# google-research/nerf-from-image

Measured on AMD Instinct MI355X. Metric: rendered rays/sec (128x128, 64+64 samples), higher is better.
Workload: dtype f32 (decoder MLP operands split-fp16 hi+lo, 22 bits; strict fp32: config.value_mlp_exact_fp32)

## Files before the change

nerf_from_image_amd/csrc/nfi_device.hpp:

```cpp
#pragma once
#include <hip/hip_runtime.h>
#include <stdint.h>

#ifndef NFI_RENDER_OCC
#define NFI_RENDER_OCC 2
#endif

namespace nfi {

typedef float f32x4 __attribute__((ext_vector_type(4)));
typedef unsigned int u32x4 __attribute__((ext_vector_type(4)));
typedef _Float16 f16x8 __attribute__((ext_vector_type(8)));

constexpr int kWave = 64;
constexpr int kC = 32;
constexpr int kHidden = 64;
constexpr float kLog2e = 1.4426950408889634f;
constexpr float kLn2 = 0.6931471805599453f;
constexpr float kSoftplusThr2 = 28.853900817779268f;

constexpr int kW1F = 0;
constexpr int kW2F = kW1F + 8 * 64 * 4;
constexpr int kB1F = kW2F + 4 * 64 * 4;
constexpr int kB2F = kB1F + 64;
// ... 659 lines not shown
            if (row >= 1 && row <= A) q[(row - 1) * (-SEMP)] = (unsigned short)(int)pq;
          } else {
            if (row >= 1 && row <= A) sem[n][row - 1] = e4[r] * inv;
          }
        }
      }
    } else {
      float r1 = bcast_row0(o[n].y), r2 = bcast_row0(o[n].z), r3 = bcast_row0(o[n].w);
      res[n].r = (1.0f / (1.0f + __builtin_amdgcn_exp2f(-r1))) * 2.004f - 1.002f;
      res[n].g = (1.0f / (1.0f + __builtin_amdgcn_exp2f(-r2))) * 2.004f - 1.002f;
      res[n].b = (1.0f / (1.0f + __builtin_amdgcn_exp2f(-r3))) * 2.004f - 1.002f;
    }
  }
}

__device__ __forceinline__ void split_f16x8(const float (&x)[8], f16x8& hi, f16x8& lo) {
  typedef float f32x2 __attribute__((ext_vector_type(2)));
#pragma unroll
  for (int i = 0; i < 4; ++i) {
    auto h = __builtin_amdgcn_cvt_pkrtz(x[2 * i], x[2 * i + 1]);
    float r0, r1;
    const uint32_t hb = __builtin_bit_cast(uint32_t, h);
    asm("v_fma_mix_f32 %0, -%1, 1.0, %2 op_sel:[0,0,0] op_sel_hi:[1,0,0]" : "=v"(r0) : "v"(hb), "v"(x[2 * i]));
    asm("v_fma_mix_f32 %0, -%1, 1.0, %2 op_sel:[1,0,0] op_sel_hi:[1,0,0]" : "=v"(r1) : "v"(hb), "v"(x[2 * i + 1]));
    auto l = __builtin_amdgcn_cvt_pkrtz(r0, r1);
    hi[2 * i] = h[0]; hi[2 * i + 1] = h[1];
    lo[2 * i] = l[0]; lo[2 * i + 1] = l[1];
  }
}

// ... 53 lines not shown
    const f16x8 al = __builtin_bit_cast(f16x8, w1t[((0 * 2 + kk) * 2 + 1) * 64 + lane]);
    const f16x8 bh = __builtin_bit_cast(f16x8, w1t[((1 * 2 + kk) * 2 + 0) * 64 + lane]);
    const f16x8 bl = __builtin_bit_cast(f16x8, w1t[((1 * 2 + kk) * 2 + 1) * 64 + lane]);
    const f32x4 zero = {0.0f, 0.0f, 0.0f, 0.0f};
    G[kk][0] = __builtin_amdgcn_mfma_f32_16x16x32_f16(al, sh, zero, 0, 0, 0);
    G[kk][1] = __builtin_amdgcn_mfma_f32_16x16x32_f16(bl, sh, zero, 0, 0, 0);
    G[kk][0] = __builtin_amdgcn_mfma_f32_16x16x32_f16(ah, sl, G[kk][0], 0, 0, 0);
    G[kk][1] = __builtin_amdgcn_mfma_f32_16x16x32_f16(bh, sl, G[kk][1], 0, 0, 0);
    G[kk][0] = __builtin_amdgcn_mfma_f32_16x16x32_f16(ah, sh, G[kk][0], 0, 0, 0);
    G[kk][1] = __builtin_amdgcn_mfma_f32_16x16x32_f16(bh, sh, G[kk][1], 0, 0, 0);
  }
  const f32x4 G0 = G[0][0] + G[1][0], G1 = G[0][1] + G[1][1];
  Gout0 = G0; Gout1 = G1;
}

template <bool ATT, int N, int PREC, int SEMP = 0, bool NRM = false>
__device__ __forceinline__ void tile_mlp(const FieldParams& P, int lane, const float (&feat)[N][8],
                                         const float (&outside)[N], float* const (&sem)[N], TileOut (&res)[N],
                                         f32x4 (&Gout)[N][2]) {
  const int g = lane >> 4;
  const f32x4* ldsv = reinterpret_cast<const f32x4*>(P.lds);
  f32x4 o[N];
  if constexpr (PREC == 1) {
    const u32x4* ldsu = reinterpret_cast<const u32x4*>(P.lds);
    f16x8 fh[N], fl[N];
#pragma unroll
    for (int n = 0; n < N; ++n) split_f16x8(feat[n], fh[n], fl[n]);
    f32x4 acc1[N][4];
#pragma unroll
    for (int nt = 0; nt < 4; ++nt) {
      const f32x4 b = ldsv[(kB1F >> 2) + g * 4 + nt];
      const f16x8 wh = __builtin_bit_cast(f16x8, ldsu[(kW1H_lds >> 2) + (nt * 2 + 0) * 64 + lane]);
      const f16x8 wl = __builtin_bit_cast(f16x8, ldsu[(kW1H_lds >> 2) + (nt * 2 + 1) * 64 + lane]);
#pragma unroll
      for (int n = 0; n < N; ++n) acc1[n][nt] = __builtin_amdgcn_mfma_f32_16x16x32_f16(wh, fh[n], b, 0, 0, 0);
#pragma unroll
      for (int n = 0; n < N; ++n) acc1[n][nt] = __builtin_amdgcn_mfma_f32_16x16x32_f16(wh, fl[n], acc1[n][nt], 0, 0, 0);
// ... 76 lines not shown
    for (int n = 0; n < N; ++n) { o0[n] = b2; o1[n] = f32x4{0.0f, 0.0f, 0.0f, 0.0f}; }
#pragma unroll
    for (int nt = 0; nt < 4; ++nt) {
      const f32x4 w = ldsv[(kW2F >> 2) + nt * 64 + lane];
#pragma unroll
      for (int n = 0; n < N; ++n) {
        o0[n] = __builtin_amdgcn_mfma_f32_16x16x4f32(w.x, acc1[n][nt][0], o0[n], 0, 0, 0);
        o1[n] = __builtin_amdgcn_mfma_f32_16x16x4f32(w.y, acc1[n][nt][1], o1[n], 0, 0, 0);
        o0[n] = __builtin_amdgcn_mfma_f32_16x16x4f32(w.z, acc1[n][nt][2], o0[n], 0, 0, 0);
        o1[n] = __builtin_amdgcn_mfma_f32_16x16x4f32(w.w, acc1[n][nt][3], o1[n], 0, 0, 0);
      }
    }
#pragma unroll
    for (int n = 0; n < N; ++n) o[n] = o0[n] + o1[n];
  }

  tile_epilogue<ATT, N, SEMP>(P, lane, o, outside, sem, res);
}
template <bool ATT, int N, int PREC, int SEMP = 0>
__device__ __forceinline__ void tile_mlp(const FieldParams& P, int lane, const float (&feat)[N][8],
                                         const float (&outside)[N], float* const (&sem)[N], TileOut (&res)[N]) {
  f32x4 unused[N][2];
  tile_mlp<ATT, N, PREC, SEMP, false>(P, lane, feat, outside, sem, res, unused);
}

template <bool ATT, int N, int SEMP = 0, bool NRM = false>
__device__ __forceinline__ void tile_mlp_vd(const FieldParams& P, int lane, const float (&feat)[N][8],
                                            const f32x4 (&xr)[N][3], const float (&outside)[N], float* const (&sem)[N],
                                            TileOut (&res)[N], f32x4 (&Gout)[N][2]) {
  const int g = lane >> 4;
  const f32x4* ldsv = reinterpret_cast<const f32x4*>(P.lds);
  f32x4 acc1[N][4];
#pragma unroll
  for (int nt = 0; nt < 4; ++nt) {
    const f32x4 b = ldsv[(kVdB1F >> 2) + g * 4 + nt];
#pragma unroll
    for (int n = 0; n < N; ++n) acc1[n][nt] = b;
  }
#pragma unroll
  for (int s = 0; s < 8; ++s) {
    const f32x4 w = ldsv[(kVdW1F >> 2) + s * 64 + lane];
#pragma unroll
    for (int n = 0; n < N; ++n) {
      acc1[n][0] = __builtin_amdgcn_mfma_f32_16x16x4f32(w.x, feat[n][s], acc1[n][0], 0, 0, 0);
// ... 28 lines not shown
    for (int n = 0; n < N; ++n) o2[n][t] = b;
  }
#pragma unroll
  for (int nt = 0; nt < 4; ++nt)
#pragma unroll
    for (int t = 0; t < 3; ++t) {
      const f32x4 w = ldsv[(kVdW2 >> 2) + (t * 4 + nt) * 64 + lane];
#pragma unroll
      for (int n = 0; n < N; ++n) {
        o2[n][t] = __builtin_amdgcn_mfma_f32_16x16x4f32(w.x, acc1[n][nt][0], o2[n][t], 0, 0, 0);
        o2[n][t] = __builtin_amdgcn_mfma_f32_16x16x4f32(w.y, acc1[n][nt][1], o2[n][t], 0, 0, 0);
        o2[n][t] = __builtin_amdgcn_mfma_f32_16x16x4f32(w.z, acc1[n][nt][2], o2[n][t], 0, 0, 0);
        o2[n][t] = __builtin_amdgcn_mfma_f32_16x16x4f32(w.w, acc1[n][nt][3], o2[n][t], 0, 0, 0);
      }
    }
  f32x4 o[N], oB[N];
  const f32x4 b3 = ldsv[(kVdB3 >> 2) + g];
#pragma unroll
  for (int n = 0; n < N; ++n) { o[n] = b3; oB[n] = f32x4{0.0f, 0.0f, 0.0f, 0.0f}; }
#pragma unroll
  for (int t = 0; t < 3; ++t) {
    const f32x4 w = ldsv[(kVdW3 >> 2) + t * 64 + lane];
#pragma unroll
    for (int n = 0; n < N; ++n) {
      f32x4 y;
#pragma unroll
      for (int r = 0; r < 4; ++r) {
        const float v = o2[n][t][r] + xr[n][t][r];
        y[r] = (v >= 0.0f) ? v : v * 0.2f;
      }
      if (t == 0 && g == 0) y[0] = o2[n][0][0];
      o[n] = __builtin_amdgcn_mfma_f32_16x16x4f32(w.x, y[0], o[n], 0, 0, 0);
      oB[n] = __builtin_amdgcn_mfma_f32_16x16x4f32(w.y, y[1], oB[n], 0, 0, 0);
      o[n] = __builtin_amdgcn_mfma_f32_16x16x4f32(w.z, y[2], o[n], 0, 0, 0);
      oB[n] = __builtin_amdgcn_mfma_f32_16x16x4f32(w.w, y[3], oB[n], 0, 0, 0);
    }
  }
#pragma unroll
  for (int n = 0; n < N; ++n) o[n] = o[n] + oB[n];
  tile_epilogue<ATT, N, SEMP>(P, lane, o, outside, sem, res);
}

struct SampleOut {
  float sdf, sigma, r, g, b;
  float nx, ny, nz;
};

template <int TEX, bool ATT, bool SKIP, int PREC = 0, bool VD = false, int SEMP = 0, bool NRM = false>
__device__ __forceinline__ SampleOut field_wave(const FieldParams& P, float scene_range, int lane, float px, float py,
                                                float pz, bool valid, float* sem_base, bool* outside_flag,
                                                float* stage, unsigned long long* prof = nullptr,
                                                const float* xray = nullptr, int ray_idx = 0) {
  float qx = px / scene_range, qy = py / scene_range, qz = pz / scene_range;
  bool out = (fabsf(qx) > 1.0f) || (fabsf(qy) > 1.0f) || (fabsf(qz) > 1.0f);
  if (outside_flag) *outside_flag = out;
  int x0, y0, z0;
  float fx, fy, fz;
  plane_coord(qx, P.res_m1, P.res, x0, fx);
  plane_coord(qy, P.res_m1, P.res, y0, fy);
  plane_coord(qz, P.res_m1, P.res, z0, fz);
  if (!valid) { x0 = y0 = z0 = 0; fx = fy = fz = 0.0f; }
  const int xi = (int)((uint32_t)x0 | ((uint32_t)y0 << 10) | ((uint32_t)z0 << 20));
  int flags = (out ? 1 : 0) | (valid ? 2 : 0);
  if constexpr (NRM) {
    auto inside = [&](float q) { float u = ((q + 1.0f) / 2.0f) * P.res_m1; return (u > 0.0f && u < P.res_m1) ? 1 : 0; };
    flags |= (inside(qx) << 2) | (inside(qy) << 3) | (inside(qz) << 4);
  }
  const uint64_t live = SKIP ? __ballot(valid && !out) : __ballot(valid);
  uint32_t tm = 0;
#pragma unroll
  for (int t = 0; t < 4; ++t) tm |= (((live >> (16 * t)) & 0xFFFFull) != 0 ? 1u : 0u) << t;

  SampleOut so;
  so.sdf = 0.0f; so.sigma = 0.0f; so.r = 0.0f; so.g = 0.0f; so.b = 0.0f;
  so.nx = 0.0f; so.ny = 0.0f; so.nz = 0.0f;
  if (tm == 0) return so;
  const int j = lane & 15, g = lane >> 4;

  const int lp = lane >> 2, lq = lane & 3;
  auto gather_tile = [&](int t, float (&feat)[8]) -> int {
    const int srcL = 16 * t + lp, srcM = 16 * t + j;
    const float cfx = __shfl(fx, srcL, 64), cfy = __shfl(fy, srcL, 64), cfz = __shfl(fz, srcL, 64);
    const uint32_t cxi = (uint32_t)__shfl(xi, srcL, 64);
    const int fcur = __shfl(flags, srcM, 64);
    float featL[8];
    TileTex<TEX> T;
    tile_issue<TEX>(P, lq, cxi, T);
    tile_bilinear<TEX>(T, cfx, cfy, cfz, featL);
    __builtin_amdgcn_sched_barrier(0);
    f32x4* wr = reinterpret_cast<f32x4*>(stage + lp * 36 + lq * 4);
    wr[0] = f32x4{featL[0], featL[1], featL[2], featL[3]};
    wr[4] = f32x4{featL[4], featL[5], featL[6], featL[7]};
    wave_lds_fence();
    const f32x4* rd = reinterpret_cast<const f32x4*>(stage + j * 36 + g * 4);
    const f32x4 lo = rd[0], hi = rd[4];
    feat[0] = lo.x; feat[1] = lo.y; feat[2] = lo.z; feat[3] = lo.w;
    feat[4] = hi.x; feat[5] = hi.y; feat[6] = hi.z; feat[7] = hi.w;
    wave_lds_fence();
    __builtin_amdgcn_sched_barrier(0);
// ... 8 lines not shown
#pragma unroll
    for (int a = 0; a < 3; ++a) {
      gcoord[a] += dpp_f32<kDppQuadXor1>(0.0f, gcoord[a]);
      gcoord[a] += dpp_f32<kDppQuadXor2>(0.0f, gcoord[a]);
    }
    const int flL = __shfl(flags, 16 * t + lp, 64);
    float gx = ((flL >> 2) & 1) ? gcoord[0] : 0.0f, gy = ((flL >> 3) & 1) ? gcoord[1] : 0.0f,
          gz = ((flL >> 4) & 1) ? gcoord[2] : 0.0f;
    const float sc = ((P.res_m1 * 0.5f) / scene_range) * P.w2r0[64];
    gx *= sc; gy *= sc; gz *= sc;
    const float rn = __builtin_amdgcn_rsqf(fmaxf(fmaf(gx, gx, fmaf(gy, gy, gz * gz)), 1e-24f));
    gx *= rn; gy *= rn; gz *= rn;
    const float sx = __shfl(gx, 4 * j, 64), sy = __shfl(gy, 4 * j, 64), sz = __shfl(gz, 4 * j, 64);
    if (g == t) { so.nx = sx; so.ny = sy; so.nz = sz; }
  };
#pragma unroll 1
  while (tm != 0) {
    if constexpr (NRM) {
      int tprev = -1;
      float dL[3][8];
      f32x4 Gp1[2];
      auto normals_of_previous = [&]() {
        f32x4* wr = reinterpret_cast<f32x4*>(stage + j * 36 + g * 4);
        wr[0] = Gp1[0]; wr[4] = Gp1[1];
        wave_lds_fence();
        float gfL[8];
        {
          const f32x4* rd = reinterpret_cast<const f32x4*>(stage + lp * 36 + lq * 4);
          const f32x4 lo = rd[0], hi = rd[4];
          gfL[0] = lo.x; gfL[1] = lo.y; gfL[2] = lo.z; gfL[3] = lo.w;
          gfL[4] = hi.x; gfL[5] = hi.y; gfL[6] = hi.z; gfL[7] = hi.w;
        }
        wave_lds_fence();
// ... 37 lines not shown
        {
          f32x4* wr = reinterpret_cast<f32x4*>(stage + lp * 36 + lq * 4);
          wr[0] = f32x4{featL[0], featL[1], featL[2], featL[3]};
          wr[4] = f32x4{featL[4], featL[5], featL[6], featL[7]};
          wave_lds_fence();
          const f32x4* rd = reinterpret_cast<const f32x4*>(stage + j * 36 + g * 4);
          const f32x4 lo = rd[0], hi = rd[4];
          feat1[0][0] = lo.x; feat1[0][1] = lo.y; feat1[0][2] = lo.z; feat1[0][3] = lo.w;
          feat1[0][4] = hi.x; feat1[0][5] = hi.y; feat1[0][6] = hi.z; feat1[0][7] = hi.w;
          wave_lds_fence();
        }
        __builtin_amdgcn_sched_barrier(0);
        __builtin_amdgcn_s_setprio(0);
        const float outs1[1] = {(f1 & 1) ? 1.0f : 0.0f};
        float* const sems1[1] = {(sem_base && (f1 & 2)) ? sem_col(t) : nullptr};
        TileOut to1[1];
        f32x4 G1[1][2];
        if constexpr (VD) {
          static_assert(PREC == 0, "the view-direction decoder exists in exact fp32 only");
          const int r1 = __shfl(ray_idx, 16 * t + j, 64);
          f32x4 xr1[1][3];
#pragma unroll
          for (int c3 = 0; c3 < 3; ++c3) xr1[0][c3] = *reinterpret_cast<const f32x4*>(xray + (size_t)r1 * kRayFeatPad + 16 * c3 + 4 * g);
          tile_mlp_vd<ATT, 1, SEMP, true>(P, lane, feat1, xr1, outs1, sems1, to1, G1);
        } else {
          tile_mlp<ATT, 1, PREC, SEMP, true>(P, lane, feat1, outs1, sems1, to1, G1);
        }
        Gp1[0] = G1[0][0]; Gp1[1] = G1[0][1];
        tprev = t;
        if (g == t) { so.sdf = to1[0].sdf; so.sigma = to1[0].sigma; so.r = to1[0].r; so.g = to1[0].g; so.b = to1[0].b; }
      }
      if (tprev >= 0) normals_of_previous();
      return so;
    }
    unsigned long long c0 = prof ? __builtin_readcyclecounter() : 0;
    const int ta = __builtin_ctz(tm);
    tm &= tm - 1;
    const bool pair = tm != 0;
    const int tb = pair ? __builtin_ctz(tm) : ta;
    tm &= tm - 1;
    float feat[2][8];
    __builtin_amdgcn_s_setprio(3);
    const int fa = gather_tile(ta, feat[0]);
    int fb = fa;
    if (pair) {
      fb = gather_tile(tb, feat[1]);
    } else {
#pragma unroll
      for (int s8 = 0; s8 < 8; ++s8) feat[1][s8] = feat[0][s8];
    }
    unsigned long long c2 = prof ? __builtin_readcyclecounter() : 0;
    __builtin_amdgcn_s_setprio(0);
    const float outs[2] = {(fa & 1) ? 1.0f : 0.0f, (fb & 1) ? 1.0f : 0.0f};
    float* const sems[2] = {(sem_base && (fa & 2)) ? sem_col(ta) : nullptr, (sem_base && pair && (fb & 2)) ? sem_col(tb) : nullptr};
    TileOut to[2];
    f32x4 Gp[2][2];
    if constexpr (VD) {
      static_assert(PREC == 0, "the view-direction decoder exists in exact fp32 only");
      const int ra = __shfl(ray_idx, 16 * ta + j, 64), rb = __shfl(ray_idx, 16 * tb + j, 64);
      f32x4 xr[2][3];
#pragma unroll
      for (int t = 0; t < 3; ++t) {
        xr[0][t] = *reinterpret_cast<const f32x4*>(xray + (size_t)ra * kRayFeatPad + 16 * t + 4 * g);
        xr[1][t] = *reinterpret_cast<const f32x4*>(xray + (size_t)rb * kRayFeatPad + 16 * t + 4 * g);
      }
      tile_mlp_vd<ATT, 2, SEMP, false>(P, lane, feat, xr, outs, sems, to, Gp);
    } else {
      tile_mlp<ATT, 2, PREC, SEMP, false>(P, lane, feat, outs, sems, to, Gp);
    }
    if (g == ta) { so.sdf = to[0].sdf; so.sigma = to[0].sigma; so.r = to[0].r; so.g = to[0].g; so.b = to[0].b; }
    if (pair && g == tb) { so.sdf = to[1].sdf; so.sigma = to[1].sigma; so.r = to[1].r; so.g = to[1].g; so.b = to[1].b; }
    if (prof) {
      asm volatile("" :: "v"(so.sigma), "v"(so.r));
      unsigned long long c3 = __builtin_readcyclecounter();
      prof[1] += c2 - c0; prof[2] += c3 - c2; prof[3] += pair ? 2 : 1;
    }
  }
  return so;
}

template <int SPL>
__device__ __forceinline__ void ray_weights(const float (&sigma)[SPL], const float (&t)[SPL], int n, float dnorm,
                                            int lane, float (&w)[SPL], float (&T)[SPL]) {
  float tn[SPL], om[SPL], alpha[SPL];
  next_elem<SPL>(t, tn, lane);
#pragma unroll
  for (int j = 0; j < SPL; ++j) {
    int e = j * 64 + lane;
    float delta = (e < n - 1) ? (tn[j] - t[j]) : 0.0f;
    delta = delta * dnorm;
// ... 28 lines not shown
```

nerf_from_image_amd/csrc/nfi_kernels.hip:

```cpp
#include "nfi_device.hpp"
#include "../../include/nfi_hip.h"
#include "nfi_host.hpp"

#include <algorithm>
#include <cstddef>
#include <cstdio>
#include <cstring>

using namespace nfi;

thread_local char nfi_err_buf[256] = "";
extern "C" const char* nfi_last_error(void) { return nfi_err_buf; }
extern "C" int nfi_version(void) { return 102; }


constexpr int kP2tPixels = 256, kP2tPitch = 288;
template <int TEX>
__global__ __launch_bounds__(256) void planes_to_texels_kernel(const float* __restrict__ planes, void* __restrict__ texels,
                                                               int hw) {
  __shared__ __attribute__((aligned(16))) float tile[kC][kP2tPitch];
  const int img = blockIdx.y;
  const int px0 = blockIdx.x * kP2tPixels;
  const float* src = planes + (size_t)img * kC * hw;
  {
// ... 430 lines not shown
  int64_t total = a->n_rays * a->n_samples;
  hipLaunchKernelGGL(stratified_kernel, dim3((unsigned)((total + 255) / 256)), dim3(256), 0, (hipStream_t)stream, *a);
  return check_launch("stratified_points");
}

struct FieldKernelParams {
  const float* points; int64_t P;
  const void* texels; int res; int tex;
  const float* image; int A; const float* att;
  int use_sdf; const float* beta; const float* alpha; float scene_range;
  float* sigma; float* rgb; float* sdf; float* sem; uint8_t* outside;
  const float* xray; int spr;
  int layout;
};

template <int TEX, bool ATT, bool VD = false, int PREC = 0>
__global__ __launch_bounds__(256) void field_query_kernel(FieldKernelParams k) {
  constexpr int kImg = VD ? kVdImageFloats : kLdsImageFloats;
  __shared__ __attribute__((aligned(16))) float lds[kImg + 64];
  __shared__ __attribute__((aligned(16))) float stages[4][16 * 36];
  const int scene = blockIdx.y;
  stage_field_lds(lds, k.image, k.att ? k.att + (size_t)scene * k.A * 3 : nullptr, k.A, kImg);
  if (PREC == 1) {
    __syncthreads();
    for (int i = threadIdx.x; i < kB1F; i += blockDim.x) lds[i] = k.image[kW1H + i];
  }
  __syncthreads();
  const size_t tb = TEX == 0 ? 128 : 64;
  const char* tex_scene = reinterpret_cast<const char*>(k.texels) + (size_t)scene * 3 * k.res * k.res * tb;
  FieldParams P = make_field_params(tex_scene, k.res, TEX, k.A, k.use_sdf, k.beta, k.alpha, lds, kImg, k.layout);
  const int lane = lane_id();
  const int wave = threadIdx.x >> 6;
  const int64_t n_chunks = (k.P + 63) / 64;
  const float* xray_scene = VD ? k.xray + (size_t)scene * (size_t)(k.P / k.spr) * kRayFeatPad : nullptr;
  for (int64_t chunk = (int64_t)blockIdx.x * 4 + wave; chunk < n_chunks; chunk += (int64_t)gridDim.x * 4) {
    int64_t p = chunk * 64 + lane;
    bool valid = p < k.P;
    size_t gi = (size_t)scene * k.P + (valid ? p : 0);
    float px = 0.0f, py = 0.0f, pz = 0.0f;
    if (valid) { px = k.points[gi * 3]; py = k.points[gi * 3 + 1]; pz = k.points[gi * 3 + 2]; }
    bool out;
    float* sem = k.sem ? k.sem + ((size_t)scene * k.P + chunk * 64) * k.A : nullptr;
    SampleOut so = field_wave<TEX, ATT, false, PREC, VD>(P, k.scene_range, lane, px, py, pz, valid, sem, &out, stages[wave],
                                                      nullptr, xray_scene, VD && valid ? (int)(p / k.spr) : 0);
    if (valid) {
      k.sigma[gi] = so.sigma;
      k.rgb[gi * 3] = so.r; k.rgb[gi * 3 + 1] = so.g; k.rgb[gi * 3 + 2] = so.b;
      if (k.sdf) k.sdf[gi] = so.sdf;
      if (k.outside) k.outside[gi] = out ? 1 : 0;
    }
  }
}

static int field_check_call(const nfi_field_args* a) {
  REQUIRE(a && a->points && a->sigma && a->rgb, "field_query: null pointer");
  REQUIRE(a->n_scenes > 0 && a->points_per_scene > 0, "field_query: bad shape");
  int rc = check_field_common(a->texels, a->plane_res, a->texel_dtype, a->decoder_image, a->n_attention,
                              a->attention_values, a->use_sdf, a->beta, a->alpha, a->texel_layout);
  if (rc) return rc;
// ... 986 lines not shown
    if (ends) { nxt = got; return; }
    a = got;
  }
  cur = nxt = a;
}

template <int TEX, bool ATT, int OCC, int MODE, int PREC, bool VD = false>
__global__ __launch_bounds__(256, OCC) void render_fwd_kernel(RenderKernelParams k) {
  constexpr bool TAPS = MODE == kRenderTaps, PROF = MODE == kRenderProf, TERM = MODE == kRenderTerm;
  constexpr bool EXTRA = MODE == kRenderExtra || MODE == kRenderNormals, NRM = MODE == kRenderNormals;
  constexpr int SEMP = (EXTRA && ATT) ? kSemPitch : 0;
  constexpr int kImg = VD ? kVdImageFloats : kLdsImageFloats;
  __shared__ __attribute__((aligned(16))) float lds[kImg];
  __shared__ __attribute__((aligned(16))) float vfs[4][64];
  __shared__ WaveSlab slabs[4];
  if constexpr (NRM) stage_normal_operands(nfi_dyn_lds, k.image, VD ? kVdW1F : kW1F, VD ? kVdW2 : kW2F);
  ClockProbe clock;
  clock.start(k);
  stage_decoder_image<PREC, kImg>(lds, k.image);
  const int lane = lane_id();
  const int wave = threadIdx.x >> 6;
  WaveSlab& slab = slabs[wave];
  float* vf = vfs[wave];
  const int S = k.S;
  const bool valid = lane < S;
  const float fill_near = ordered_key_inv(~k.reduce[0]), fill_far = ordered_key_inv(k.reduce[1]);
  const float bg = k.white ? 1.0f : 0.0f;
  const uint32_t n_rays = (uint32_t)k.n_scenes * (uint32_t)k.hw;

  FieldParams P = make_field_params(k.texels, k.res, TEX, k.A, k.use_sdf, k.beta, k.alpha, lds, kImg, k.layout);
  P.vf = vf;
  P.w1t = nfi_dyn_lds; P.w2r0 = nfi_dyn_lds + kW1TFloats;
  int cur_scene = -1;

  float* semT = nullptr;
  if constexpr (SEMP > 0) {
    if (k.semantics) {
      semT = nfi_dyn_lds + (NRM ? kNrmLdsFloats : 0) + wave * (k.A * kSemPitch);
// ... 35 lines not shown
      cur_scene = scene;
      enter_scene<TEX>(P, k, vf, scene, lane);
    }
    const float ox = in.ox, oy = in.oy, oz = in.oz, dx = in.dx, dy = in.dy, dz = in.dz;
    float near = in.near, far = in.far;
    finish_planes((hitb & 1) != 0, fill_near, fill_far, near, far);
    const float dnorm = norm3(dx, dy, dz);
    const size_t rs = (size_t)ray * (size_t)k.tap_stride;

    float tc = 0.0f;
    if (valid) tc = stratified_depth(near, far, lane, S, in.noise, k.noise_c != nullptr);
    MergeIn c;
    float ncx = 0.0f, ncy = 0.0f, ncz = 0.0f, nfx = 0.0f, nfy = 0.0f, nfz = 0.0f;
    unsigned long long t1 = PROF ? __builtin_readcyclecounter() : 0;
    {
      SampleOut q = field_wave<TEX, ATT, true, PREC, VD, SEMP, NRM>(P, k.scene_range, lane, ox + dx * tc, oy + dy * tc, oz + dz * tc,
                                                                    valid, semT, nullptr, &slab.srt[0][0], PROF ? pc : nullptr,
                                                                    k.xray, (int)ray);
      c.t = tc; c.sigma = q.sigma; c.r = q.r; c.g = q.g; c.b = q.b;
      if constexpr (NRM) { ncx = q.nx; ncy = q.ny; ncz = q.nz; }
    }
    int n = S;
    int rank_c = lane, rank_f = 0;
    unsigned long long t2 = PROF ? __builtin_readcyclecounter() : 0, t3 = t2, t4 = t2, t5 = t2;
    if (k.fine) {
      ResampleTaps rt;
      float tf = resample_ray(slab, c.sigma, tc, S, dnorm, in.u, lane, TERM ? &rt : nullptr);
      MergeIn f;
      if (PROF) { asm volatile("" :: "v"(tf)); t3 = __builtin_readcyclecounter(); }
      if constexpr (TERM) {
        const uint64_t dm = __ballot(valid && rt.T < k.term_eps);
        float t_dead = INFINITY;
        if (dm) t_dead = bits2f((uint32_t)__builtin_amdgcn_readlane((int)f2bits(tc), (int)__builtin_ctzll(dm)));
        const bool live = valid && tf <= t_dead;
        const uint64_t lm = __ballot(live);
        const int nl = __builtin_popcountll(lm);
        const int nb = __builtin_popcountll(lm & ((1ull << lane) - 1ull));
        const int pos = live ? nb : nl + (lane - nb);
        wave_lds_fence();
        slab.cdf[pos] = tf;
        wave_lds_fence();
        tf = slab.cdf[lane];
        wave_lds_fence();
        const bool vl = lane < nl;
        SampleOut q = field_wave<TEX, ATT, true, PREC, VD>(P, k.scene_range, lane, ox + dx * tf, oy + dy * tf, oz + dz * tf, vl,
                                                           nullptr, nullptr, &slab.srt[0][0], nullptr, k.xray, (int)ray);
        f.t = tf; f.sigma = vl ? q.sigma : 0.0f; f.r = vl ? q.r : 0.0f; f.g = vl ? q.g : 0.0f; f.b = vl ? q.b : 0.0f;
      } else {
        SampleOut q = field_wave<TEX, ATT, true, PREC, VD, SEMP, NRM>(P, k.scene_range, lane, ox + dx * tf, oy + dy * tf, oz + dz * tf,
                                                                      valid, semT ? semT + 64 : nullptr, nullptr, &slab.srt[0][0],
                                                                      PROF ? pc : nullptr, k.xray, (int)ray);
        f.t = tf; f.sigma = q.sigma; f.r = q.r; f.g = q.g; f.b = q.b;
        if constexpr (NRM) { nfx = q.nx; nfy = q.ny; nfz = q.nz; }
      }
      if constexpr (TAPS) {
        if (valid) store_sample_tap(k.t_fine, k.sigma_fine, k.rgb_fine, rs + lane, tf, f.sigma, f.r, f.g, f.b);
      }
      n = 2 * S;
      if (PROF) t4 = __builtin_readcyclecounter();
      merge_pair_scatter(slab, c, f, S, lane, rank_c, rank_f);
      if (PROF) t5 = __builtin_readcyclecounter();
    } else {
      if (valid) { slab.srt[0][lane] = c.t; slab.srt[1][lane] = c.sigma; slab.srt[2][lane] = c.r; slab.srt[3][lane] = c.g; slab.srt[4][lane] = c.b; }
      wave_lds_fence();
    }
    float w[2];
// ... 135 lines not shown

      float tc[2], sc[2], rc[2], gc[2], bc[2];
      bool val[2];
#pragma unroll
      for (int j = 0; j < 2; ++j) {
        const int e = j * 64 + lane;
        val[j] = e < S;
        const float nz = (k.noise_c && val[j]) ? k.noise_c[rs + e] : 0.0f;
        tc[j] = val[j] ? stratified_depth(near, far, e, S, nz, k.noise_c != nullptr) : 0.0f;
      }
      float nrm[4][3];
#pragma unroll
      for (int j = 0; j < 4; ++j) nrm[j][0] = nrm[j][1] = nrm[j][2] = 0.0f;
#pragma unroll
      for (int j = 0; j < 2; ++j) {
        SampleOut q = field_wave<TEX, ATT, true, PREC, VD, SEMP, NRM>(P, k.scene_range, lane, ox + dx * tc[j], oy + dy * tc[j],
                                                                      oz + dz * tc[j], val[j], sem_col(j * 64), nullptr,
                                                                      stage, nullptr, k.xray, (int)ray);
        sc[j] = q.sigma; rc[j] = q.r; gc[j] = q.g; bc[j] = q.b;
        if constexpr (NRM) { nrm[j][0] = q.nx; nrm[j][1] = q.ny; nrm[j][2] = q.nz; }
      }
      int n = S;
      float dep[4], sig[4], cr[4], cg[4], cb[4];
      int eidx[4], rank[4];
#pragma unroll
      for (int j = 0; j < 2; ++j) {
        dep[j] = tc[j]; sig[j] = sc[j]; cr[j] = rc[j]; cg[j] = gc[j]; cb[j] = bc[j];
        eidx[j] = val[j] ? j * 64 + lane : 0x7fffffff;
        dep[2 + j] = sig[2 + j] = cr[2 + j] = cg[2 + j] = cb[2 + j] = 0.0f;
        eidx[2 + j] = 0x7fffffff;
        rank[j] = j * 64 + lane; rank[2 + j] = 0;
      }
      if (k.fine) {
// ... 17 lines not shown
          const int b0 = __builtin_popcountll(lm0 & below), b1 = __builtin_popcountll(lm1 & below);
          const int p0 = l0 ? b0 : nl + (lane - b0);
          const int p1 = l1 ? n0 + b1 : nl + (64 - n0) + (lane - b1);
          wave_lds_fence();
          slab.cdf[p0] = tf[0];
          slab.cdf[p1] = tf[1];
          wave_lds_fence();
          tf[0] = slab.cdf[lane];
          tf[1] = slab.cdf[64 + lane];
          wave_lds_fence();
          vfine[0] = lane < nl;
          vfine[1] = 64 + lane < nl;
        }
#pragma unroll
        for (int j = 0; j < 2; ++j) {
          SampleOut q = field_wave<TEX, ATT, true, PREC, VD, SEMP, NRM>(P, k.scene_range, lane, ox + dx * tf[j], oy + dy * tf[j],
                                                                        oz + dz * tf[j], vfine[j], sem_col(128 + j * 64),
                                                                        nullptr, stage, nullptr, k.xray, (int)ray);
          if (TERM && !vfine[j]) { q.sigma = 0.0f; q.r = 0.0f; q.g = 0.0f; q.b = 0.0f; }
          if constexpr (NRM) { nrm[2 + j][0] = q.nx; nrm[2 + j][1] = q.ny; nrm[2 + j][2] = q.nz; }
          dep[2 + j] = tf[j]; sig[2 + j] = q.sigma; cr[2 + j] = q.r; cg[2 + j] = q.g; cb[2 + j] = q.b;
          eidx[2 + j] = val[j] ? S + j * 64 + lane : 0x7fffffff;
          if constexpr (TAPS) {
            if (val[j]) store_sample_tap(k.t_fine, k.sigma_fine, k.rgb_fine, ts + j * 64 + lane, tf[j], q.sigma, q.r, q.g, q.b);
          }
        }
        n = 2 * S;
        wave_lds_fence();
        if (!merge_pair_scatter_wide(slab, dep, sig, cr, cg, cb, S, lane, rank))
          merge_scatter<4>(slab, dep, sig, cr, cg, cb, eidx, n, rank);
      } else {
        wave_lds_fence();
#pragma unroll
// ... 116 lines not shown
        enter_scene<TEX>(P, k, vf, scene, lane);
      }
      const size_t r3 = (size_t)ray * 3;
      const float ox = k.ro[r3], oy = k.ro[r3 + 1], oz = k.ro[r3 + 2];
      const float dx = k.rd[r3], dy = k.rd[r3 + 1], dz = k.rd[r3 + 2];
      float near = k.near_raw[ray], far = k.far_raw[ray];
      finish_planes((hitb & 1) != 0, fill_near, fill_far, near, far);
      const float dnorm = norm3(dx, dy, dz);
      const size_t rs = (size_t)ray * S;
#pragma unroll 1
      for (int j = 0; j < slots; ++j) {
        const int e = j * 64 + lane;
        const bool val = e < S;
        const float nz = (k.noise_c && val) ? k.noise_c[rs + e] : 0.0f;
        const float t = val ? stratified_depth(near, far, e, S, nz, k.noise_c != nullptr) : 0.0f;
        SampleOut q = field_wave<TEX, ATT, true, PREC, VD>(P, k.scene_range, lane, ox + dx * t, oy + dy * t, oz + dz * t, val,
                                                           nullptr, nullptr, slab.stage, nullptr, k.xray, (int)ray);
        if (val) {
          slab.srt[0][e] = t; slab.srt[1][e] = q.sigma; slab.srt[2][e] = q.r; slab.srt[3][e] = q.g; slab.srt[4][e] = q.b;
          store_sample_tap(k.t_coarse, k.sigma_coarse, k.rgb_coarse, ts + e, t, q.sigma, q.r, q.g, q.b);
        }
      }
      wave_lds_fence();
      float w[NS];
      CompositeOut o = composite_slab<NS>(slab, S, dnorm, k.white, lane, w);
      if (lane == 0) {
        store_pixel(k, ray, o.r, o.g, o.b, o.depth, o.mask);
        if (k.near_plane) k.near_plane[ray] = near;
        if (k.far_plane) k.far_plane[ray] = far;
      }
      if (k.weights || k.t_sorted) store_sorted_taps<NS>(k, slab, w, ray, S, lane);
      if (k.perm) {
// ... 289 lines not shown
```

Before: 148.6 million.

## Park MLP tile outputs in LDS and run a per-sample epilogue once per wave

For plain attention rendering without view direction, the decoder MLP's raw MFMA outputs for each tile are written to a per-wave LDS table instead of running the softmax/sigmoid epilogue per tile pair. After all tiles finish, each lane reads its own sample's row column and computes sigma, attention softmax colour and semantic weights in one pass. This replaces the cross-lane broadcast and repeated per-tile epilogue work with a transpose through LDS, at the cost of extra LDS space and two wave fences per field query.

```diff
diff --git a/nerf_from_image_amd/csrc/nfi_device.hpp b/nerf_from_image_amd/csrc/nfi_device.hpp
--- a/nerf_from_image_amd/csrc/nfi_device.hpp
+++ b/nerf_from_image_amd/csrc/nfi_device.hpp
@@ -697,6 +697,111 @@
   }
 }
 
+constexpr int kOutPitch = 64 + 4;
+constexpr int kOutLastRow = 14;
+template <bool ATT>
+constexpr int kOutTabFloats = (ATT ? 16 : 4) * kOutPitch;
+
+template <bool ATT>
+__device__ __forceinline__ void park_tile_outputs(float* otab, int lane, int t, const f32x4& o) {
+  const int g = lane >> 4, j = lane & 15;
+  auto* q = (__attribute__((address_space(3))) float*)otab + (4 * g) * kOutPitch + 16 * t + j;
+  if (ATT || g == 0) {
+    q[0] = o.x; q[kOutPitch] = o.y; q[2 * kOutPitch] = o.z; q[3 * kOutPitch] = o.w;
+  }
+}
+
+template <bool ATT, int SEMP>
+__device__ __forceinline__ void sample_epilogue(const FieldParams& P, int lane, const float* otab, bool outside, bool live,
+                                                float* sem, float& o_sdf, float& o_sigma, float& o_r, float& o_g, float& o_b) {
+  const auto* tb = (const __attribute__((address_space(3))) float*)otab + lane;
+  const float sdf = tb[0];
+  const float outs = outside ? 1.0f : 0.0f;
+  float sigma, cr, cg, cb;
+  if (P.use_sdf) {
+    float e = __builtin_amdgcn_exp2f(fabsf(sdf) * P.neg_log2e_over_beta);
+    float sgn = (sdf < 0.0f) ? 0.5f : ((sdf > 0.0f) ? -0.5f : 0.0f);
+    float cdf = 0.5f + sgn * (1.0f - e);
+    sigma = P.inv_alpha * (cdf * (1.0f - outs));
+  } else {
+    float d = sdf - 1.0f;
+    float sp = (d > 20.0f) ? d : log1pf(__expf(d));
+    sigma = sp * (1.0f - outs);
+  }
+  if constexpr (ATT) {
+    const int A = P.n_attention;
+    float x[16], e16[16];
+    float m = -INFINITY;
+#pragma unroll
+    for (int gi = 0; gi < 4; ++gi) {
+      if (4 * gi <= A) {
+#pragma unroll
+        for (int r = 0; r < 4; ++r) {
+          const int row = 4 * gi + r;
+          if (row == 0 || row > kOutLastRow) continue;
+          x[row] = tb[row * kOutPitch];
+          m = (row <= A) ? fmaxf(m, x[row]) : m;
+        }
+      }
+    }
+    const f32x4* vf = reinterpret_cast<const f32x4*>(P.vf);
+    float seg[4], srg[4], sgg[4], sbg[4];
+#pragma unroll
+    for (int gi = 0; gi < 4; ++gi) {
+      float se = 0.0f, sr = 0.0f, sg = 0.0f, sb = 0.0f;
+      if (4 * gi <= A) {
+#pragma unroll
+        for (int r = 0; r < 4; ++r) {
+          const int row = 4 * gi + r;
+          if (row == 0 || row > kOutLastRow) continue;
+          const float e = (row <= A) ? __builtin_amdgcn_exp2f(x[row] - m) : 0.0f;
+          e16[row] = e;
+          const f32x4 v = vf[row];
+          se += e;
+          sr = fmaf(e, v.x, sr);
+          sg = fmaf(e, v.y, sg);
+          sb = fmaf(e, v.z, sb);
+        }
+      }
+      seg[gi] = se; srg[gi] = sr; sgg[gi] = sg; sbg[gi] = sb;
+    }
+    const float se = (seg[0] + seg[1]) + (seg[2] + seg[3]), sr = (srg[0] + srg[1]) + (srg[2] + srg[3]),
+                sg = (sgg[0] + sgg[1]) + (sgg[2] + sgg[3]), sb = (sbg[0] + sbg[1]) + (sbg[2] + sbg[3]);
+    float inv = __builtin_amdgcn_rcpf(se);
+    inv = inv * (2.0f - se * inv);
+    cr = sr * inv; cg = sg * inv; cb = sb * inv;
+    if (sem && live) {
+#pragma unroll
+      for (int gi = 0; gi < 4; ++gi) {
+        if (4 * gi <= A) {
+#pragma unroll
+          for (int r = 0; r < 4; ++r) {
+            const int row = 4 * gi + r;
+            if (row == 0 || row > kOutLastRow) continue;
+            if constexpr (SEMP > 0) {
+              auto* q = (__attribute__((address_space(3))) float*)sem;
+              if (row <= A) q[(row - 1) * SEMP] = e16[row] * inv;
+            } else if constexpr (SEMP < 0) {
+              auto* q = (__attribute__((address_space(3))) unsigned short*)sem;
+              const float pq = fminf(__builtin_rintf(e16[row] * inv * 65535.0f), 65535.0f);
+              if (row <= A) q[(row - 1) * (-SEMP)] = (unsigned short)(int)pq;
+            } else {
+              if (row <= A) sem[row - 1] = e16[row] * inv;
+            }
+          }
+        }
+      }
+    }
+  } else {
+    const float r1 = tb[kOutPitch], r2 = tb[2 * kOutPitch], r3 = tb[3 * kOutPitch];
+    cr = (1.0f / (1.0f + __builtin_amdgcn_exp2f(-r1))) * 2.004f - 1.002f;
+    cg = (1.0f / (1.0f + __builtin_amdgcn_exp2f(-r2))) * 2.004f - 1.002f;
+    cb = (1.0f / (1.0f + __builtin_amdgcn_exp2f(-r3))) * 2.004f - 1.002f;
+  }
+  o_sdf = live ? sdf : 0.0f; o_sigma = live ? sigma : 0.0f;
+  o_r = live ? cr : 0.0f; o_g = live ? cg : 0.0f; o_b = live ? cb : 0.0f;
+}
+
 __device__ __forceinline__ void split_f16x8(const float (&x)[8], f16x8& hi, f16x8& lo) {
   typedef float f32x2 __attribute__((ext_vector_type(2)));
 #pragma unroll
@@ -780,13 +885,11 @@
   Gout0 = G0; Gout1 = G1;
 }
 
-template <bool ATT, int N, int PREC, int SEMP = 0, bool NRM = false>
-__device__ __forceinline__ void tile_mlp(const FieldParams& P, int lane, const float (&feat)[N][8],
-                                         const float (&outside)[N], float* const (&sem)[N], TileOut (&res)[N],
+template <int N, int PREC, bool NRM = false>
+__device__ __forceinline__ void tile_mlp(const FieldParams& P, int lane, const float (&feat)[N][8], f32x4 (&o)[N],
                                          f32x4 (&Gout)[N][2]) {
   const int g = lane >> 4;
   const f32x4* ldsv = reinterpret_cast<const f32x4*>(P.lds);
-  f32x4 o[N];
   if constexpr (PREC == 1) {
     const u32x4* ldsu = reinterpret_cast<const u32x4*>(P.lds);
     f16x8 fh[N], fl[N];
@@ -893,20 +996,11 @@
 #pragma unroll
     for (int n = 0; n < N; ++n) o[n] = o0[n] + o1[n];
   }
-
-  tile_epilogue<ATT, N, SEMP>(P, lane, o, outside, sem, res);
-}
-template <bool ATT, int N, int PREC, int SEMP = 0>
-__device__ __forceinline__ void tile_mlp(const FieldParams& P, int lane, const float (&feat)[N][8],
-                                         const float (&outside)[N], float* const (&sem)[N], TileOut (&res)[N]) {
-  f32x4 unused[N][2];
-  tile_mlp<ATT, N, PREC, SEMP, false>(P, lane, feat, outside, sem, res, unused);
-}
-
-template <bool ATT, int N, int SEMP = 0, bool NRM = false>
+}
+
+template <int N, bool NRM = false>
 __device__ __forceinline__ void tile_mlp_vd(const FieldParams& P, int lane, const float (&feat)[N][8],
-                                            const f32x4 (&xr)[N][3], const float (&outside)[N], float* const (&sem)[N],
-                                            TileOut (&res)[N], f32x4 (&Gout)[N][2]) {
+                                            const f32x4 (&xr)[N][3], f32x4 (&o)[N], f32x4 (&Gout)[N][2]) {
   const int g = lane >> 4;
   const f32x4* ldsv = reinterpret_cast<const f32x4*>(P.lds);
   f32x4 acc1[N][4];
@@ -965,7 +1059,7 @@
         o2[n][t] = __builtin_amdgcn_mfma_f32_16x16x4f32(w.w, acc1[n][nt][3], o2[n][t], 0, 0, 0);
       }
     }
-  f32x4 o[N], oB[N];
+  f32x4 oB[N];
   const f32x4 b3 = ldsv[(kVdB3 >> 2) + g];
 #pragma unroll
   for (int n = 0; n < N; ++n) { o[n] = b3; oB[n] = f32x4{0.0f, 0.0f, 0.0f, 0.0f}; }
@@ -989,7 +1083,6 @@
   }
 #pragma unroll
   for (int n = 0; n < N; ++n) o[n] = o[n] + oB[n];
-  tile_epilogue<ATT, N, SEMP>(P, lane, o, outside, sem, res);
 }
 
 struct SampleOut {
@@ -997,10 +1090,10 @@
   float nx, ny, nz;
 };
 
-template <int TEX, bool ATT, bool SKIP, int PREC = 0, bool VD = false, int SEMP = 0, bool NRM = false>
+template <int TEX, bool ATT, bool SKIP, int PREC, bool VD, int SEMP, bool NRM, bool OTAB>
 __device__ __forceinline__ SampleOut field_wave(const FieldParams& P, float scene_range, int lane, float px, float py,
                                                 float pz, bool valid, float* sem_base, bool* outside_flag,
-                                                float* stage, unsigned long long* prof = nullptr,
+                                                float* stage, float* otab, unsigned long long* prof = nullptr,
                                                 const float* xray = nullptr, int ray_idx = 0) {
   float qx = px / scene_range, qy = py / scene_range, qz = pz / scene_range;
   bool out = (fabsf(qx) > 1.0f) || (fabsf(qy) > 1.0f) || (fabsf(qz) > 1.0f);
@@ -1026,6 +1119,7 @@
   so.sdf = 0.0f; so.sigma = 0.0f; so.r = 0.0f; so.g = 0.0f; so.b = 0.0f;
   so.nx = 0.0f; so.ny = 0.0f; so.nz = 0.0f;
   if (tm == 0) return so;
+  const uint32_t tm_live = tm;
   const int j = lane & 15, g = lane >> 4;
 
   const int lp = lane >> 2, lq = lane & 3;
@@ -1033,7 +1127,7 @@
     const int srcL = 16 * t + lp, srcM = 16 * t + j;
     const float cfx = __shfl(fx, srcL, 64), cfy = __shfl(fy, srcL, 64), cfz = __shfl(fz, srcL, 64);
     const uint32_t cxi = (uint32_t)__shfl(xi, srcL, 64);
-    const int fcur = __shfl(flags, srcM, 64);
+    const int fcur = OTAB ? 0 : __shfl(flags, srcM, 64);
     float featL[8];
     TileTex<TEX> T;
     tile_issue<TEX>(P, lq, cxi, T);
@@ -1072,9 +1166,9 @@
     const float sx = __shfl(gx, 4 * j, 64), sy = __shfl(gy, 4 * j, 64), sz = __shfl(gz, 4 * j, 64);
     if (g == t) { so.nx = sx; so.ny = sy; so.nz = sz; }
   };
-#pragma unroll 1
-  while (tm != 0) {
-    if constexpr (NRM) {
+  if constexpr (NRM) {
+    static_assert(!OTAB, "the normal map's one-tile-per-turn schedule runs the per-tile epilogue");
+    {
       int tprev = -1;
       float dL[3][8];
       f32x4 Gp1[2];
@@ -1142,7 +1236,7 @@
         __builtin_amdgcn_s_setprio(0);
         const float outs1[1] = {(f1 & 1) ? 1.0f : 0.0f};
         float* const sems1[1] = {(sem_base && (f1 & 2)) ? sem_col(t) : nullptr};
-        TileOut to1[1];
+        f32x4 o1[1];
         f32x4 G1[1][2];
         if constexpr (VD) {
           static_assert(PREC == 0, "the view-direction decoder exists in exact fp32 only");
@@ -1150,17 +1244,23 @@
           f32x4 xr1[1][3];
 #pragma unroll
           for (int c3 = 0; c3 < 3; ++c3) xr1[0][c3] = *reinterpret_cast<const f32x4*>(xray + (size_t)r1 * kRayFeatPad + 16 * c3 + 4 * g);
-          tile_mlp_vd<ATT, 1, SEMP, true>(P, lane, feat1, xr1, outs1, sems1, to1, G1);
+          tile_mlp_vd<1, true>(P, lane, feat1, xr1, o1, G1);
         } else {
-          tile_mlp<ATT, 1, PREC, SEMP, true>(P, lane, feat1, outs1, sems1, to1, G1);
+          tile_mlp<1, PREC, true>(P, lane, feat1, o1, G1);
+        }
+        {
+          TileOut to1[1];
+          tile_epilogue<ATT, 1, SEMP>(P, lane, o1, outs1, sems1, to1);
+          if (g == t) { so.sdf = to1[0].sdf; so.sigma = to1[0].sigma; so.r = to1[0].r; so.g = to1[0].g; so.b = to1[0].b; }
         }
         Gp1[0] = G1[0][0]; Gp1[1] = G1[0][1];
         tprev = t;
-        if (g == t) { so.sdf = to1[0].sdf; so.sigma = to1[0].sigma; so.r = to1[0].r; so.g = to1[0].g; so.b = to1[0].b; }
       }
       if (tprev >= 0) normals_of_previous();
-      return so;
-    }
+    }
+  }
+#pragma unroll 1
+  while (!NRM && tm != 0) {
     unsigned long long c0 = prof ? __builtin_readcyclecounter() : 0;
     const int ta = __builtin_ctz(tm);
     tm &= tm - 1;
@@ -1180,8 +1280,9 @@
     unsigned long long c2 = prof ? __builtin_readcyclecounter() : 0;
     __builtin_amdgcn_s_setprio(0);
     const float outs[2] = {(fa & 1) ? 1.0f : 0.0f, (fb & 1) ? 1.0f : 0.0f};
-    float* const sems[2] = {(sem_base && (fa & 2)) ? sem_col(ta) : nullptr, (sem_base && pair && (fb & 2)) ? sem_col(tb) : nullptr};
-    TileOut to[2];
+    float* const sems[2] = {(!OTAB && sem_base && (fa & 2)) ? sem_col(ta) : nullptr,
+                            (!OTAB && sem_base && pair && (fb & 2)) ? sem_col(tb) : nullptr};
+    f32x4 o[2];
     f32x4 Gp[2][2];
     if constexpr (VD) {
       static_assert(PREC == 0, "the view-direction decoder exists in exact fp32 only");
@@ -1192,16 +1293,40 @@
         xr[0][t] = *reinterpret_cast<const f32x4*>(xray + (size_t)ra * kRayFeatPad + 16 * t + 4 * g);
         xr[1][t] = *reinterpret_cast<const f32x4*>(xray + (size_t)rb * kRayFeatPad + 16 * t + 4 * g);
       }
-      tile_mlp_vd<ATT, 2, SEMP, false>(P, lane, feat, xr, outs, sems, to, Gp);
+      tile_mlp_vd<2, false>(P, lane, feat, xr, o, Gp);
     } else {
-      tile_mlp<ATT, 2, PREC, SEMP, false>(P, lane, feat, outs, sems, to, Gp);
-    }
-    if (g == ta) { so.sdf = to[0].sdf; so.sigma = to[0].sigma; so.r = to[0].r; so.g = to[0].g; so.b = to[0].b; }
-    if (pair && g == tb) { so.sdf = to[1].sdf; so.sigma = to[1].sigma; so.r = to[1].r; so.g = to[1].g; so.b = to[1].b; }
+      tile_mlp<2, PREC, false>(P, lane, feat, o, Gp);
+    }
+    if constexpr (OTAB) {
+      park_tile_outputs<ATT>(otab, lane, ta, o[0]);
+      if (pair) park_tile_outputs<ATT>(otab, lane, tb, o[1]);
+      if (prof) asm volatile("" :: "v"(o[0].x), "v"(o[1].x));
+    } else {
+      TileOut to[2];
+      tile_epilogue<ATT, 2, SEMP>(P, lane, o, outs, sems, to);
+      if (g == ta) { so.sdf = to[0].sdf; so.sigma = to[0].sigma; so.r = to[0].r; so.g = to[0].g; so.b = to[0].b; }
+      if (pair && g == tb) { so.sdf = to[1].sdf; so.sigma = to[1].sigma; so.r = to[1].r; so.g = to[1].g; so.b = to[1].b; }
+      if (prof) asm volatile("" :: "v"(so.sigma), "v"(so.r));
+    }
+    if (prof) {
+      unsigned long long c3 = __builtin_readcyclecounter();
+      prof[1] += c2 - c0; prof[2] += c3 - c2; prof[3] += pair ? 2 : 1;
+    }
+  }
+  if constexpr (OTAB) {
+    unsigned long long c4 = prof ? __builtin_readcyclecounter() : 0;
+    wave_lds_fence();
+    const bool live = valid && ((tm_live >> (lane >> 4)) & 1u);
+    float* sem_mine = nullptr;
+    if (sem_base) {
+      if constexpr (SEMP < 0) sem_mine = reinterpret_cast<float*>(reinterpret_cast<unsigned short*>(sem_base) + lane);
+      else sem_mine = sem_base + (size_t)lane * sem_pt;
+    }
+    sample_epilogue<ATT, SEMP>(P, lane, otab, out, live, sem_mine, so.sdf, so.sigma, so.r, so.g, so.b);
+    wave_lds_fence();
     if (prof) {
       asm volatile("" :: "v"(so.sigma), "v"(so.r));
-      unsigned long long c3 = __builtin_readcyclecounter();
-      prof[1] += c2 - c0; prof[2] += c3 - c2; prof[3] += pair ? 2 : 1;
+      prof[2] += __builtin_readcyclecounter() - c4;
     }
   }
   return so;
diff --git a/nerf_from_image_amd/csrc/nfi_kernels.hip b/nerf_from_image_amd/csrc/nfi_kernels.hip
--- a/nerf_from_image_amd/csrc/nfi_kernels.hip
+++ b/nerf_from_image_amd/csrc/nfi_kernels.hip
@@ -468,6 +468,7 @@
   int layout;
 };
 
+static_assert(kOutLastRow == NFI_MAX_ATTENTION, "sample_epilogue reads rows 1 .. NFI_MAX_ATTENTION of the output table");
 template <int TEX, bool ATT, bool VD = false, int PREC = 0>
 __global__ __launch_bounds__(256) void field_query_kernel(FieldKernelParams k) {
   constexpr int kImg = VD ? kVdImageFloats : kLdsImageFloats;
@@ -495,8 +496,9 @@
     if (valid) { px = k.points[gi * 3]; py = k.points[gi * 3 + 1]; pz = k.points[gi * 3 + 2]; }
     bool out;
     float* sem = k.sem ? k.sem + ((size_t)scene * k.P + chunk * 64) * k.A : nullptr;
-    SampleOut so = field_wave<TEX, ATT, false, PREC, VD>(P, k.scene_range, lane, px, py, pz, valid, sem, &out, stages[wave],
-                                                      nullptr, xray_scene, VD && valid ? (int)(p / k.spr) : 0);
+    SampleOut so = field_wave<TEX, ATT, false, PREC, VD, 0, false, false>(P, k.scene_range, lane, px, py, pz, valid, sem, &out,
+                                                                          stages[wave], nullptr, nullptr, xray_scene,
+                                                                          VD && valid ? (int)(p / k.spr) : 0);
     if (valid) {
       k.sigma[gi] = so.sigma;
       k.rgb[gi * 3] = so.r; k.rgb[gi * 3 + 1] = so.g; k.rgb[gi * 3 + 2] = so.b;
@@ -1513,6 +1515,8 @@
   __shared__ __attribute__((aligned(16))) float lds[kImg];
   __shared__ __attribute__((aligned(16))) float vfs[4][64];
   __shared__ WaveSlab slabs[4];
+  constexpr bool OTAB = MODE == kRenderPlain && ATT && !VD;
+  __shared__ __attribute__((aligned(16))) float otabs[4][OTAB ? kOutTabFloats<ATT> : 4];
   if constexpr (NRM) stage_normal_operands(nfi_dyn_lds, k.image, VD ? kVdW1F : kW1F, VD ? kVdW2 : kW2F);
   ClockProbe clock;
   clock.start(k);
@@ -1521,6 +1525,7 @@
   const int wave = threadIdx.x >> 6;
   WaveSlab& slab = slabs[wave];
   float* vf = vfs[wave];
+  float* otab = otabs[wave];
   const int S = k.S;
   const bool valid = lane < S;
   const float fill_near = ordered_key_inv(~k.reduce[0]), fill_far = ordered_key_inv(k.reduce[1]);
@@ -1586,8 +1591,8 @@
     float ncx = 0.0f, ncy = 0.0f, ncz = 0.0f, nfx = 0.0f, nfy = 0.0f, nfz = 0.0f;
     unsigned long long t1 = PROF ? __builtin_readcyclecounter() : 0;
     {
-      SampleOut q = field_wave<TEX, ATT, true, PREC, VD, SEMP, NRM>(P, k.scene_range, lane, ox + dx * tc, oy + dy * tc, oz + dz * tc,
-                                                                    valid, semT, nullptr, &slab.srt[0][0], PROF ? pc : nullptr,
+      SampleOut q = field_wave<TEX, ATT, true, PREC, VD, SEMP, NRM, OTAB>(P, k.scene_range, lane, ox + dx * tc, oy + dy * tc, oz + dz * tc,
+                                                                    valid, semT, nullptr, &slab.srt[0][0], otab, PROF ? pc : nullptr,
                                                                     k.xray, (int)ray);
       c.t = tc; c.sigma = q.sigma; c.r = q.r; c.g = q.g; c.b = q.b;
       if constexpr (NRM) { ncx = q.nx; ncy = q.ny; ncz = q.nz; }
@@ -1615,13 +1620,14 @@
         tf = slab.cdf[lane];
         wave_lds_fence();
         const bool vl = lane < nl;
-        SampleOut q = field_wave<TEX, ATT, true, PREC, VD>(P, k.scene_range, lane, ox + dx * tf, oy + dy * tf, oz + dz * tf, vl,
-                                                           nullptr, nullptr, &slab.srt[0][0], nullptr, k.xray, (int)ray);
+        SampleOut q = field_wave<TEX, ATT, true, PREC, VD, 0, false, OTAB>(P, k.scene_range, lane, ox + dx * tf, oy + dy * tf,
+                                                                           oz + dz * tf, vl, nullptr, nullptr, &slab.srt[0][0],
+                                                                           otab, nullptr, k.xray, (int)ray);
         f.t = tf; f.sigma = vl ? q.sigma : 0.0f; f.r = vl ? q.r : 0.0f; f.g = vl ? q.g : 0.0f; f.b = vl ? q.b : 0.0f;
       } else {
-        SampleOut q = field_wave<TEX, ATT, true, PREC, VD, SEMP, NRM>(P, k.scene_range, lane, ox + dx * tf, oy + dy * tf, oz + dz * tf,
+        SampleOut q = field_wave<TEX, ATT, true, PREC, VD, SEMP, NRM, OTAB>(P, k.scene_range, lane, ox + dx * tf, oy + dy * tf, oz + dz * tf,
                                                                       valid, semT ? semT + 64 : nullptr, nullptr, &slab.srt[0][0],
-                                                                      PROF ? pc : nullptr, k.xray, (int)ray);
+                                                                      otab, PROF ? pc : nullptr, k.xray, (int)ray);
         f.t = tf; f.sigma = q.sigma; f.r = q.r; f.g = q.g; f.b = q.b;
         if constexpr (NRM) { nfx = q.nx; nfy = q.ny; nfz = q.nz; }
       }
@@ -1787,9 +1793,9 @@
       for (int j = 0; j < 4; ++j) nrm[j][0] = nrm[j][1] = nrm[j][2] = 0.0f;
 #pragma unroll
       for (int j = 0; j < 2; ++j) {
-        SampleOut q = field_wave<TEX, ATT, true, PREC, VD, SEMP, NRM>(P, k.scene_range, lane, ox + dx * tc[j], oy + dy * tc[j],
-                                                                      oz + dz * tc[j], val[j], sem_col(j * 64), nullptr,
-                                                                      stage, nullptr, k.xray, (int)ray);
+        SampleOut q = field_wave<TEX, ATT, true, PREC, VD, SEMP, NRM, false>(P, k.scene_range, lane, ox + dx * tc[j], oy + dy * tc[j],
+                                                                             oz + dz * tc[j], val[j], sem_col(j * 64), nullptr,
+                                                                             stage, nullptr, nullptr, k.xray, (int)ray);
         sc[j] = q.sigma; rc[j] = q.r; gc[j] = q.g; bc[j] = q.b;
         if constexpr (NRM) { nrm[j][0] = q.nx; nrm[j][1] = q.ny; nrm[j][2] = q.nz; }
       }
@@ -1837,9 +1843,9 @@
         }
 #pragma unroll
         for (int j = 0; j < 2; ++j) {
-          SampleOut q = field_wave<TEX, ATT, true, PREC, VD, SEMP, NRM>(P, k.scene_range, lane, ox + dx * tf[j], oy + dy * tf[j],
-                                                                        oz + dz * tf[j], vfine[j], sem_col(128 + j * 64),
-                                                                        nullptr, stage, nullptr, k.xray, (int)ray);
+          SampleOut q = field_wave<TEX, ATT, true, PREC, VD, SEMP, NRM, false>(P, k.scene_range, lane, ox + dx * tf[j], oy + dy * tf[j],
+                                                                               oz + dz * tf[j], vfine[j], sem_col(128 + j * 64),
+                                                                               nullptr, stage, nullptr, nullptr, k.xray, (int)ray);
           if (TERM && !vfine[j]) { q.sigma = 0.0f; q.r = 0.0f; q.g = 0.0f; q.b = 0.0f; }
           if constexpr (NRM) { nrm[2 + j][0] = q.nx; nrm[2 + j][1] = q.ny; nrm[2 + j][2] = q.nz; }
           dep[2 + j] = tf[j]; sig[2 + j] = q.sigma; cr[2 + j] = q.r; cg[2 + j] = q.g; cb[2 + j] = q.b;
@@ -1986,8 +1992,9 @@
         const bool val = e < S;
         const float nz = (k.noise_c && val) ? k.noise_c[rs + e] : 0.0f;
         const float t = val ? stratified_depth(near, far, e, S, nz, k.noise_c != nullptr) : 0.0f;
-        SampleOut q = field_wave<TEX, ATT, true, PREC, VD>(P, k.scene_range, lane, ox + dx * t, oy + dy * t, oz + dz * t, val,
-                                                           nullptr, nullptr, slab.stage, nullptr, k.xray, (int)ray);
+        SampleOut q = field_wave<TEX, ATT, true, PREC, VD, 0, false, false>(P, k.scene_range, lane, ox + dx * t, oy + dy * t,
+                                                                            oz + dz * t, val, nullptr, nullptr, slab.stage,
+                                                                            nullptr, nullptr, k.xray, (int)ray);
         if (val) {
           slab.srt[0][e] = t; slab.srt[1][e] = q.sigma; slab.srt[2][e] = q.r; slab.srt[3][e] = q.g; slab.srt[4][e] = q.b;
           store_sample_tap(k.t_coarse, k.sigma_coarse, k.rgb_coarse, ts + e, t, q.sigma, q.r, q.g, q.b);
```

Result: faster. 153.1 million (median of 6 runs) (+3.0%).
